# Cyan4973/FiniteStateEntropy

Hardware: AMD Instinct MI355X
Metric: MB/s encode+decode per GPU on 32KB probagen blocks; bit-exact vs CPU ref (higher is better)
Workload: dtype u8; 1 GPU; probagen Proba14, 100000 x 32KB blocks per GPU, FSE encode+decode (one-shot calls at the reference's default limits: tableLog 11, decode maxLog 12), bit-exact check; blocks_per_gpu=100000, block_bytes=32768, codec=fse, parity=fse: roundtrip-all-blocks

## Files before the change

### finitestateentropy_amd/csrc/fse_decode.hip

```cpp
#include "internal.h"
#include <atomic>

#include "bitreader.h"

#ifndef FSE_SYM_L1
#define FSE_SYM_L1 1
#endif
#ifndef FSE_DEC_RING
#define FSE_DEC_RING 64
#endif
#define FSE_IN_RING 256
#define FSE_IN_RING_LOG 8
#define FSE_IN_CHUNK 64
#define FSE_IN_LANES (FSE_IN_CHUNK / 4)
#define FSE_IN_MIRROR 16
#ifndef FSE_CHECK_EVERY
#define FSE_CHECK_EVERY 16
#endif
#ifndef FSE_PHASE_UNROLL
#define FSE_PHASE_UNROLL 16
#endif
#define FSE_FINISH_EVERY 2
#ifndef FSE_DEC_LDS_KB
#define FSE_DEC_LDS_KB 160
// ... 240 lines not shown
                nextOff -= FSE_IN_CHUNK;
                pend = 0;
                if (nextOff >= 0 && nextOff + 4 <= SgK) pend = gbl_load_u32(igK + nextOff);
            }
        }
#pragma unroll
        for (int l = 0; l < FSE_SRV_G; ++l) {
            if (!((fm >> l) & 1ull)) continue;
            const u32 cnt = srv_rl(avail, l), fp_g = srv_rl(fpos, l);
            const gbl_u8_ptr tg = (gbl_u8_ptr)(uintptr_t)srv_rl64(tabBits, l);
            if ((u32)lane < cnt) {
                u32 ri = fp_g + (u32)lane;
                ri = ri >= FSE_DEC_RING ? ri - FSE_DEC_RING : ri;
                const u32* const rw = (const u32*)(ldsb + (size_t)(g0 + l) * slotBytes + ringOff) + 4u * (ri >> 1) + (ri & 1u);
                uint2 rec; rec.x = rw[0]; rec.y = rw[2];
                const u32 x0 = __builtin_amdgcn_ubfe(rec.x, 1u, a.ldsLog), x1 = __builtin_amdgcn_ubfe(rec.x, 17u, a.ldsLog);
                const u32 x2 = __builtin_amdgcn_ubfe(rec.y, 1u, a.ldsLog), x3 = __builtin_amdgcn_ubfe(rec.y, 17u, a.ldsLog);
#if FSE_SYM_L1
                yq[l][0] = tg[x0]; yq[l][2] = tg[x1]; yq[l][1] = tg[x2]; yq[l][3] = tg[x3];
#else
                if (CALLER) {
                    yq[l][0] = __hip_atomic_load(tg + x0, __ATOMIC_RELAXED, __HIP_MEMORY_SCOPE_AGENT); yq[l][2] = __hip_atomic_load(tg + x1, __ATOMIC_RELAXED, __HIP_MEMORY_SCOPE_AGENT);
                    yq[l][1] = __hip_atomic_load(tg + x2, __ATOMIC_RELAXED, __HIP_MEMORY_SCOPE_AGENT); yq[l][3] = __hip_atomic_load(tg + x3, __ATOMIC_RELAXED, __HIP_MEMORY_SCOPE_AGENT);
                } else { yq[l][0] = tg[x0]; yq[l][2] = tg[x1]; yq[l][1] = tg[x2]; yq[l][3] = tg[x3]; }
#endif
            }
        }
        if (wantFlush) { ctl_store(&ctl->srvFlushed, it); }
#pragma unroll
        for (int l = 0; l < FSE_SRV_G; ++l) {
            if (!((fm >> l) & 1ull)) continue;
            const u32 cnt = srv_rl(avail, l), fl_g = srv_rl(flushed, l);
            gbl_u8_w_ptr const og = (gbl_u8_w_ptr)(uintptr_t)(srv_rl64(outBits, l) + 4ull * fl_g);
            if ((u32)lane < cnt) {
                const u32 w = yq[l][0] | (yq[l][1] << 8) | (yq[l][2] << 16) | (yq[l][3] << 24);
                gbl_store_u32(og + 4u * lane, w);
            }
        }
        if (wantFlush) { fpos += it - flushed; fpos = fpos >= FSE_DEC_RING ? fpos - FSE_DEC_RING : fpos; flushed = it; }
        TIMING(const unsigned long long sB = __builtin_readcyclecounter(); sBusy += sB - sA; sA = sB; ++nBusy;);
    }
    TIMING(if (lane == 0 && g0 == 0) { atomicAdd(&g_decTiming[5], sBusy); atomicAdd(&g_decTiming[6], sIdle); });
    if (CALLER) fse_scratch_slot_done(a, flagsSh, lane);
}

struct FseCellsRef { const u32* cells;
    DEV void get(u32 st, u32& ns, u32& nb, u32& sym) const { const u32 c = cells[st]; ns = c & 0xFFFFu; sym = (c >> 16) & 0xFFu; nb = c >> 24; } };
struct FseCellsCompact { const u16* A; const u8* syms;
    DEV void get(u32 st, u32& ns, u32& nb, u32& sym) const { const u32 c = A[st]; ns = c & 0xFFFu; nb = c >> 12; sym = syms[st]; } };
struct FseCellsRev { const u16* A; const u8* syms; u32 tl, cellShift;
    DEV void get(u32 st, u32& ns, u32& nb, u32& sym) const { const u32 i = __brev(st) >> (32u - tl); const u32 c = A[i]; nb = c & 31u; ns = __brev(c >> cellShift) >> (32u - tl); sym = syms[i]; } };
template <class Cells>
DEV u32 fse_tail_step(const Cells& t, u32& state, BitReader& r, bool fast)
{
    u32 ns, nb, sym;
    t.get(state, ns, nb, sym);
    const u32 low = fast ? r.read_fast(nb) : r.read(nb);
    state = ns + low;
    return sym;
}
template <class Cells>
DEV size_t fse_tail(const Cells& t, u32 s1, u32 s2, BitReader& r, u8* out, long op, long omax, bool fast)
{
    for (;;) {
        const int st = r.reload();
        if (!((st == BR_UNFINISHED) & (op < omax - 3))) break;
        u32 w = fse_tail_step(t, s1, r, fast);
        w |= fse_tail_step(t, s2, r, fast) << 8;
        w |= fse_tail_step(t, s1, r, fast) << 16;
        w |= fse_tail_step(t, s2, r, fast) << 24;
        __builtin_memcpy(out + op, &w, 4);
        op += 4;
    }
    for (;;) {
        if (op > omax - 2) return FERR(dstSize_tooSmall);
        out[op++] = (u8)fse_tail_step(t, s1, r, fast);
        if (r.reload() == BR_OVERFLOW) { out[op++] = (u8)fse_tail_step(t, s2, r, fast); return (size_t)op; }
        if (op > omax - 2) return FERR(dstSize_tooSmall);
        out[op++] = (u8)fse_tail_step(t, s2, r, fast);
        if (r.reload() == BR_OVERFLOW) { out[op++] = (u8)fse_tail_step(t, s1, r, fast); return (size_t)op; }
    }
}

template <bool FAST, bool TIMED, bool CALLER, bool VIEW = false>
__global__ __launch_bounds__(FSE_DEC_THREADS) void k_fse_decode(FseDecArgs a)
{
    extern __shared__ __attribute__((aligned(16))) u32 lds[];
    const int tid = threadIdx.x, lane = tid & 63, wave = tid >> 6;
    unsigned long long tBorn = 0, wBorn = 0;
    (void)tBorn; (void)wBorn;
    TIMING(tBorn = __builtin_readcyclecounter(); wBorn = wall_clock64(););
    const size_t first = (size_t)blockIdx.x * a.G;
    static_assert(FSE_DBINS % 4 == 0, "the bin lengths are read as 16-byte vectors");
    size_t nTot = a.nBlocks, q0 = first;
    u32 bin0 = 0, cnt0 = 0xFFFFFFFFu;
    if (a.count) {
        uint4 cv[FSE_DBINS / 4];
#pragma unroll
        for (u32 i = 0; i < FSE_DBINS / 4; ++i) cv[i] = ((const uint4*)a.count)[i];
        u64 before = 0;
        bool found = false;
#pragma unroll
        for (u32 i = 0; i < FSE_DBINS; ++i) {
            const uint4 v = cv[i >> 2];
            const u32 c = (i & 3u) == 0 ? v.x : (i & 3u) == 1 ? v.y : (i & 3u) == 2 ? v.z : v.w;
            const bool here = !found & (((u64)first < before + c) | (i == FSE_DBINS - 1));
            bin0 = here ? i : bin0; q0 = here ? (size_t)((u64)first - before) : q0; cnt0 = here ? c : cnt0;
            found |= here;
            before += c;
        }
        nTot = (size_t)before;
    }
    if (first >= nTot) return;
    auto slotBlock = [&](size_t g) -> size_t {
        if (!a.list) return first + g;
        size_t q = q0 + g; u32 i = bin0;
        if (q >= cnt0) {
            while (i < FSE_DBINS - 1) { const u32 c = a.count[i]; if (q < c) break; q -= c; ++i; }
        }
        return a.list[(size_t)i * a.nBlocks + q];
    };
    u8* const lds8 = (u8*)lds;
    const u32 tabStride = 2u << a.ldsLog;
    DecCtl* const ctlAll = (DecCtl*)(lds8 + (size_t)a.G * tabStride);
    u8* const ldsb = (u8*)ctlAll + (size_t)a.G * sizeof(DecCtl);
    const u32 slotBytes = a.slotU32 * 4u;
    const u32 ringOff = 0;
    const u32 inOff = FSE_DEC_RING * 8;

    u32* const flagsSh = (u32*)(ldsb + (size_t)a.G * slotBytes);
    if (tid < 6 || tid == 7) flagsSh[tid] = 0;
    const bool decWave = wave < FSE_DEC_WAVES;
    u8* const tlSh = (u8*)(flagsSh + 8);
    if (CALLER) {
        __syncthreads();
        bool mine = false;
        if (tid >= 64 && tid < 64 + a.G) {
            const size_t g = (size_t)tid - 64;
            u32 tl = 0xFFu;
            if (first + g < nTot) {
                const size_t bi = slotBlock(g);
                if (!(a.onlyDeclined && a.results[bi] != FSE_DECLINED)) {
                    const u32 t0 = a.dtables[bi * a.dtStrideU32] & 0xFFFFu;
                    if (t0 <= a.ldsLog && t0 >= a.tlMin) tl = t0;
                    else if (t0 > a.maxTableLog && a.tlMin == 0 && !a.onlyDeclined) a.results[bi] = FERR(tableLog_tooLarge);
                }
            }
            tlSh[g] = (u8)tl;
            mine = tl != 0xFFu;
        }
        if (mine) flagsSh[1] = 1u;
        u32 slot = 0;
        if (tid == 0) slot = fse_scratch_slot_claim(a, flagsSh);
        __syncthreads();
        if (!flagsSh[1]) {
            if (tid == 0) __hip_atomic_fetch_and(a.slotBitmap + (slot >> 5), ~(1u << (slot & 31u)), __ATOMIC_RELEASE, __HIP_MEMORY_SCOPE_AGENT);
            return;
        }
    }
    else __syncthreads();
    u8* const symSlot = CALLER ? a.symScratch + (size_t)flagsSh[6] * a.scratchSlotBytes : nullptr;
    {   u64 badBits = 0, declBits = 0; bool anyNb0 = false;
        if (!CALLER) {
            const size_t nTab = nTot - first < (size_t)a.G ? nTot - first : (size_t)a.G;
            if (tabStride >= 1024u) {
                const u32 ppt = tabStride >> 10;
                const u32 nPieces = (u32)nTab * ppt;
                for (u32 p = (u32)wave; p < nPieces; p += FSE_DEC_THREADS / 64) {
                    const u32 g = p / ppt, k = p - g * ppt;
                    const size_t bi = slotBlock(g);
                    const u8* const src = (const u8*)(a.atab + (bi << a.maxTableLog)) + 1024u * k + 16u * (u32)lane;
                    __builtin_amdgcn_global_load_lds((const __attribute__((address_space(1))) void*)src,
                                                     (__attribute__((address_space(3))) void*)(lds8 + 1024u * p), 16, 0, 0);
                }
            }
            else {
            uint4* const dstv = (uint4*)lds8;
            const u32 vptLog = a.ldsLog - 3u;
            const u32 nvec = (u32)nTab << vptLog;
            constexpr u32 MAXV = (FSE_MAXG * 512u / 16u + FSE_DEC_THREADS - 1) / FSE_DEC_THREADS;
            uint4 buf[MAXV];
#pragma unroll
            for (u32 k = 0; k < MAXV; ++k) {
                const u32 idx = tid + k * FSE_DEC_THREADS;
                if (idx < nvec) {
                    const size_t sl = first + (idx >> vptLog);
                    const size_t bi = slotBlock(sl - first);
                    buf[k] = ((const uint4*)(a.atab + (bi << a.maxTableLog)))[idx & ((1u << vptLog) - 1u)];
                }
            }
#pragma unroll
            for (u32 k = 0; k < MAXV; ++k) { const u32 idx = tid + k * FSE_DEC_THREADS; if (idx < nvec) dstv[idx] = buf[k]; }
            }
            if (!FAST) for (size_t g = 0; g < nTab; ++g) {
                const u32 st = a.meta[slotBlock(g)].state; anyNb0 |= st != 0 && !(st & 2u); }
        }
        else {
            const size_t nTab = nTot - first < (size_t)a.G ? nTot - first : (size_t)a.G;
            constexpr u32 QL = 2048u / 4u / 64u;
            if (!decWave) for (u32 g = (u32)wave - FSE_DEC_WAVES; g < (u32)nTab; g += FSE_SRV_WAVES) {
                const u32 tl = tlSh[g];
                if (tl == 0xFFu) continue;
                const u32 ts = 1u << tl;
                const u32* const t = a.dtables + slotBlock(g) * a.dtStrideU32;
                u8* const slotB = lds8 + (size_t)g * tabStride;
                u16* const A = (u16*)slotB;
                u8* const symOut = symSlot + ((size_t)g << a.ldsLog);
                bool bad = false, nbz = false;
                if (FAST && tl >= 4u) {
                    const u32 sR = 32u - tl;
                    const u32 qo[4] = { 0u, 1u << (tl - 1u), 1u << (tl - 2u), 3u << (tl - 2u) };
                    const u32 passes = ts > 2048u ? ts / 2048u : 1u;
                    u32 acc = 0, minNb = 15u;
                    uint4 cv[QL];
                    for (u32 h = 0; h < passes; ++h) {
#pragma unroll
                        for (u32 j = 0; j < QL; ++j) {
                            const u32 i0 = 2048u * h + 4u * ((u32)lane + 64u * j);
                            cv[j] = make_uint4(0, 0, 0, 0);
                            if (i0 < ts) __builtin_memcpy(&cv[j], t + 1 + i0, 16);
                        }
#pragma unroll
                        for (u32 j = 0; j < QL; ++j) {
                            const u32 i0 = 2048u * h + 4u * ((u32)lane + 64u * j);
                            if (i0 >= ts) continue;
                            const u32 r0 = __brev(i0) >> sR;
                            const u32 cw[4] = { cv[j].x, cv[j].y, cv[j].z, cv[j].w };
#pragma unroll
                            for (u32 q = 0; q < 4; ++q) {
                                const u32 c = cw[q], ns = c & 0xFFFFu, nb = c >> 24;
                                acc |= (ns >> tl) | ((tl - nb) >> 5) | (ns & ((1u << (nb & 31u)) - 1u));
                                minNb = nb < minNb ? nb : minNb;
                                slotB[r0 | qo[q]] = (u8)(c >> 16);
                            }
                        }
                    }
                    { for (u32 off = 16u * (u32)lane; off < ts; off += 1024u) { const uint4 v = *(const uint4*)(slotB + off); *(uint4*)(symOut + off) = v; } }
                    for (u32 h = 0; h < passes; ++h) {
                        if (passes > 1u) {
#pragma unroll
// ... 34 lines not shown
        if (badBits) { atomicOr(&flagsSh[2], (u32)badBits); atomicOr(&flagsSh[3], (u32)(badBits >> 32)); }
        if (declBits) { atomicOr(&flagsSh[4], (u32)declBits); atomicOr(&flagsSh[5], (u32)(declBits >> 32)); }
        if (anyNb0) atomicOr(&flagsSh[0], 1u);
    }
    const int ppw = (a.G + FSE_DEC_WAVES - 1) / FSE_DEC_WAVES;
    const int gsl = (decWave ? wave * ppw : 0) + (lane >> 1);
    const u32 half = (u32)lane & 1u, maskB = half ? ~0u : 0u;
    const bool inRange = (lane >> 1) < ppw && gsl < a.G && first + (size_t)gsl < nTot;
    const size_t b = inRange ? slotBlock((size_t)gsl) : 0;
    bool owner = decWave && inRange;
    u32 hdr = 0;
    if (owner && a.meta) { if (a.meta[b].state == 0) owner = false; else hdr = a.meta[b].hdrSize; }
    u32 tl = 0; bool fast = false;
    constexpr bool compact = !CALLER;
    const u32* const gtab = compact ? nullptr : a.dtables + (owner ? b : 0) * a.dtStrideU32;
    if (owner) {
        if (compact) { tl = a.meta[b].tableLog; fast = (a.meta[b].state & 2u) != 0; if (tl > a.ldsLog) { a.results[b] = FERR(tableLog_tooLarge); owner = false; } }
        else {
            const u32 h0 = gtab[0]; tl = h0 & 0xFFFFu; fast = (h0 >> 16) != 0;
            if (tlSh[gsl] == 0xFFu) owner = false;
        }
    }
    const u32* const cells = compact ? nullptr : gtab + 1;
    const u8* const syms = compact ? a.symtab + ((owner ? b : 0) << a.maxTableLog) : symSlot + ((size_t)(gsl < a.G ? gsl : 0) << a.ldsLog);
    const u32 ldsBase = (u32)(uintptr_t)(__attribute__((address_space(3))) u8*)lds8;
    if (ldsBase & (tabStride - 1)) __builtin_trap();
    const u32 tabOff = ldsBase + (u32)(gsl < a.G ? gsl : 0) * tabStride;
    const u16* const A = (const u16*)(lds8 + (tabOff - ldsBase));
    const u8* in = nullptr; size_t S = 0; u8* out = nullptr;
    const long omax = VIEW ? (long)a.dstCaps[owner ? b : 0] : (long)a.dstCapacity;
    long op = 0;
    BitReader r; r.base = nullptr; r.size = 0; r.at = 0; r.win = 0; r.used = 0;
    u32 s1 = 0, s2 = 0;
    if (owner) {
        in = view_ptr(a.csrc, b) + hdr;
        S = view_size(a.csrc, b) - hdr;
        out = VIEW ? a.dst + a.dstOffsets[b] : a.dst + b * a.dstStride;
        const size_t e = r.init(in, S);
        if (is_err(e)) { a.results[b] = e; owner = false; }
        else {
            s1 = r.read(tl); r.reload();
            s2 = r.read(tl); r.reload();
        }
    }

    __builtin_amdgcn_s_waitcnt(0x0f70);
    __syncthreads();
    const u64 badMask = (u64)flagsSh[2] | ((u64)flagsSh[3] << 32);
    const u64 declMask = (u64)flagsSh[4] | ((u64)flagsSh[5] << 32);
    const bool nb0 = flagsSh[0] != 0;
    if (CALLER && owner && a.declineNb0 && ((declMask >> gsl) & 1ull)) { if (half == 0) a.results[b] = FSE_DECLINED; owner = false; }

    const bool bulkOk = owner && S < (1ull << 28) && !((badMask >> gsl) & 1ull) && !(FAST && !compact && ((declMask >> gsl) & 1ull));
    const int Bstart = bulkOk ? (int)(8u * ((u32)r.at + 8u)) - (int)r.used : 0;
    const long groups0 = (omax - 3 - op + 3) / 4;
    bool can = bulkOk && (FAST ? Bstart >= 65 + 48 * (FSE_CHECK_EVERY - 1) : r.at >= 24 + 6 * FSE_CHECK_EVERY + 8) && groups0 >= FSE_CHECK_EVERY;
    bool can2 = FAST && bulkOk && Bstart >= 65 + 48 * (FSE_FINISH_EVERY - 1) && groups0 >= FSE_FINISH_EVERY;
    const bool everBulk = can || can2;
    BulkState bs; bs.q = 0; bs.bq = 0;
    {   const u32 st = half ? s2 : s1;
        bs.s = tabOff + 2u * (FAST ? __brev(st) >> (32u - (tl ? tl : 1u)) : st); }
    const u32 inA = (u32)((uintptr_t)in & 3u);
    const u32 R8 = 8u * (((u32)S + inA + 3u) & ~3u);
    u32 P = 0;
    long groups = 0;
    u32 iters = 0;
    int validLo = 0;
    if (everBulk) {
        const u32 B = 8u * ((u32)r.at + 8u + inA) - r.used;
        bs.q = 4u * (B >> 5) - 8u; bs.bq = B & 31u; P = R8 - B;
        groups = (omax - 3 - op + 3) >> 2;
        const int c0 = (int)((0 - ((uintptr_t)in - inA)) & (FSE_IN_CHUNK - 1));
        validLo = (((int)bs.q + 8 - 112 - c0) & ~(FSE_IN_CHUNK - 1)) + c0;
    }
    DecCtl* const ctl = ctlAll + (gsl < a.G ? gsl : 0);
    if (decWave && (lane >> 1) < ppw && gsl < a.G && half == 0) {
        ctl->pubIters = 0; ctl->pubPofs = everBulk ? bs.q + 8u : 0x80000000u;
        ctl->srvFlushed = 0; ctl->srvValidLo = 0x7FFFFFFF;
        ctl->initValidLo = validLo; ctl->S32 = (int)(S < (1ull << 31) ? S + inA : 0);
        const unsigned long long ib = (unsigned long long)(uintptr_t)(in - inA), ob = (unsigned long long)(uintptr_t)out, tb = (unsigned long long)(uintptr_t)syms;
        ctl->inLo = (u32)ib; ctl->inHi = (u32)(ib >> 32); ctl->outLo = (u32)ob; ctl->outHi = (u32)(ob >> 32); ctl->symLo = (u32)tb; ctl->symHi = (u32)(tb >> 32);
    }
    __syncthreads();
    if (!decWave) { fse_decode_service<TIMED, CALLER>(a, ldsb, ctlAll, slotBytes, ringOff, inOff, lane, (wave - FSE_DEC_WAVES) * FSE_SRV_G, FAST, flagsSh); return; }

    __builtin_amdgcn_s_setprio(3);
    uint2* const myRing = (uint2*)(ldsb + (size_t)(gsl < a.G ? gsl : 0) * slotBytes + ringOff) + half;
    const u32 myIn = (u32)(uintptr_t)(__attribute__((address_space(3))) u8*)(ldsb + (size_t)(gsl < a.G ? gsl : 0) * slotBytes + inOff);
    unsigned long long tRun = 0, tWait = 0, nRun = 0, nWait = 0, tA = 0, tFin = 0, nFin = 0, tInner = 0;
    (void)tRun; (void)tWait; (void)nRun; (void)nWait; (void)tA; (void)tFin; (void)nFin; (void)tInner;
    TIMING(tA = __builtin_readcyclecounter(););
    const unsigned long long tBulk0 = tA;
    (void)tBulk0;
    u32 rpos = 0;
    u64 srvNext = ctl_peek2(&ctl->srvFlushed);
    const u32 inA8 = 8u * inA;
    u32 Phead = P;
    int grp = groups > (1 << 30) ? (1 << 30) : (int)groups;
    if constexpr (FAST) {
        uint2* const dummyRing = (uint2*)(flagsSh + 32) + half;
        if ((lane >> 1) < ppw && everBulk) {
        for (;;) {
            const int lowest = (int)bs.q - 4 * ((48 * (FSE_CHECK_EVERY - 1) + 31) / 32);
            const int need = lowest > 0 ? lowest : 0;
            bool rdy;
            do {
                const u32 fl = (u32)srvNext;
                const int vlo = (int)(u32)(srvNext >> 32);
                srvNext = ctl_peek2(&ctl->srvFlushed);
                rdy = !can | ((iters + FSE_CHECK_EVERY - fl <= FSE_DEC_RING) & (need >= vlo));
                TIMING(if (!__all(rdy)) { const unsigned long long tB = __builtin_readcyclecounter(); tWait += tB - tA; ++nWait; tA = tB; });
            } while (!__all(rdy));
            if (!__any(can)) break;
            uint2* const ring = can ? myRing + rpos : dummyRing;
            u32 sN = bs.s, Pn = P, PhN = Phead;
            unsigned long long tI = 0; (void)tI;
            TIMING(tI = __builtin_readcyclecounter(););
            fse_bulk_phase_rev<FSE_CHECK_EVERY>(sN, Pn, PhN, tl + 1u, 4u, tabOff, myIn, maskB & 31u, ring);
            TIMING(tInner += __builtin_readcyclecounter() - tI;);
            bs.s = can ? sN : bs.s; P = can ? Pn : P; Phead = can ? PhN : Phead;
            const u32 adv = can ? (u32)FSE_CHECK_EVERY : 0u;
            rpos = (rpos + adv) & (FSE_DEC_RING - 1);
            iters += adv; grp -= (int)adv;
            const u32 B = R8 - P;
            bs.q = 4u * (B >> 5) - 8u;
            const u32 Bp = B - inA8;
            const bool canN = can & (Bp >= 65u + 48u * (FSE_CHECK_EVERY - 1)) & (grp >= FSE_CHECK_EVERY);
            const bool more = canN | ((Bp >= 65u + 48u * (FSE_FINISH_EVERY - 1)) & (grp >= FSE_FINISH_EVERY));
            if (can & (half == 0)) ctl_store2(&ctl->pubIters, iters, more ? bs.q + 8u : ((bs.q + 8u) | 0x80000000u));
            can = canN;
            TIMING(const unsigned long long tB = __builtin_readcyclecounter(); tRun += tB - tA; ++nRun; tA = tB;);
        }
        {   const u32 B = R8 - P; bs.bq = B & 31u;
            can2 = bulkOk & (B - inA8 >= 65u + 48u * (FSE_FINISH_EVERY - 1)) & (grp >= FSE_FINISH_EVERY); }
        can2 = can2 & bulkOk;
        for (;;) {
            const u32 fl = (u32)srvNext;
            const int vlo = (int)(u32)(srvNext >> 32);
            srvNext = ctl_peek2(&ctl->srvFlushed);
            const int lowest = (int)bs.q - 8;
            const bool rdy = !can2 | ((iters + FSE_FINISH_EVERY - fl <= FSE_DEC_RING) & ((lowest > 0 ? lowest : 0) >= vlo));
            if (!__all(rdy)) {
                TIMING(const unsigned long long tB = __builtin_readcyclecounter(); tWait += tB - tA; ++nWait; tA = tB;);
                continue;
            }
            if (!__any(can2)) break;
            uint2* const ring = can2 ? myRing + rpos : dummyRing;
            u32 sN = bs.s, Pn = P, PhN = Phead;
            fse_bulk_phase_rev<FSE_FINISH_EVERY>(sN, Pn, PhN, tl + 1u, 4u, tabOff, myIn, maskB & 31u, ring);
            bs.s = can2 ? sN : bs.s; P = can2 ? Pn : P; Phead = can2 ? PhN : Phead;
            rpos = can2 ? (rpos + FSE_FINISH_EVERY) & (FSE_DEC_RING - 1) : rpos;
            iters += can2 ? FSE_FINISH_EVERY : 0u; grp -= can2 ? FSE_FINISH_EVERY : 0;
            const u32 B = R8 - P;
            bs.q = 4u * (B >> 5) - 8u; bs.bq = B & 31u;
            const bool can2N = can2 & (B - inA8 >= 65u + 48u * (FSE_FINISH_EVERY - 1)) & (grp >= FSE_FINISH_EVERY);
            if (can2 & (half == 0)) ctl_store2(&ctl->pubIters, iters, can2N ? bs.q + 8u : ((bs.q + 8u) | 0x80000000u));
            can2 = can2N;
            TIMING(const unsigned long long tB = __builtin_readcyclecounter(); tFin += tB - tA; ++nFin; tA = tB;);
        }
        }
    } else {
    while (__any(can)) {
        const u32 fl = (u32)srvNext;
        const int vlo = (int)(u32)(srvNext >> 32);
        srvNext = ctl_peek2(&ctl->srvFlushed);
        const int lowest = (int)bs.q - (6 * FSE_CHECK_EVERY + 8);
        const bool ready = can & (iters + FSE_CHECK_EVERY - fl <= FSE_DEC_RING) & ((lowest > 0 ? lowest : 0) >= vlo);
        if (ready) {
            uint2* const ring = myRing + rpos;
            rpos = (rpos + FSE_CHECK_EVERY) & (FSE_DEC_RING - 1);
            if (nb0) fse_bulk_phase<true>(bs.s, bs.q, bs.bq, tabOff, myIn, half, maskB, ring);
            else     fse_bulk_phase<false>(bs.s, bs.q, bs.bq, tabOff, myIn, half, maskB, ring);
            iters += FSE_CHECK_EVERY; grp -= FSE_CHECK_EVERY;
            can = (bs.q >= 24u + 6u * FSE_CHECK_EVERY + 4u) & (grp >= FSE_CHECK_EVERY);
            if (half == 0) ctl_store2(&ctl->pubIters, iters, can ? bs.q + 8u : ((bs.q + 8u) | 0x80000000u));
        }
        TIMING(const unsigned long long tB = __builtin_readcyclecounter(); if (__any(ready)) { tRun += tB - tA; ++nRun; } else { tWait += tB - tA; ++nWait; } tA = tB;);
    }
    }
    TIMING(if (lane == 0) { atomicAdd(&g_decTiming[0], tRun); atomicAdd(&g_decTiming[1], tWait); atomicAdd(&g_decTiming[2], nRun); atomicAdd(&g_decTiming[3], nWait); atomicAdd(&g_decTiming[4], 1ull);
                            atomicAdd(&g_decTiming[13], tBulk0 - tBorn); atomicAdd(&g_decTiming[15], tFin); atomicAdd(&g_decTiming[10], nFin); atomicAdd(&g_decTiming[7], tInner); });
    const u32 sOther = dpp_swap(bs.s);
    const unsigned long long tBulk1 = tA;
    (void)tBulk1;
    if (owner && !half) {
    op = 4 * (long)iters;
    if (iters) {
        const u32 B = 8u * (bs.q + 8u) + bs.bq - 8u * inA;
        const u32 Bh = FAST ? R8 - Phead - 8u * inA : B;
        r.at = (size_t)((Bh + 7u) >> 3) - 8; r.used = 8u * ((u32)r.at + 8u) - B; r.win = ldg64u(in + r.at); s1 = (bs.s - tabOff) >> 1; s2 = (sOther - tabOff) >> 1;
        if (FAST) { s1 = __brev(s1) >> (32u - tl); s2 = __brev(s2) >> (32u - tl); }
    }

    size_t result;
    if (!compact) {
        if ((badMask >> gsl) & 1ull) result = fse_tail(FseCellsRef{cells}, s1, s2, r, out, op, omax, fast);
        else if (FAST)               result = fse_tail(FseCellsRev{A, syms, tl, 5u}, s1, s2, r, out, op, omax, fast);
        else                         result = fse_tail(FseCellsCompact{A, syms}, s1, s2, r, out, op, omax, fast);
    }
    else if (FAST)    result = fse_tail(FseCellsRev{A, syms, tl, 5u}, s1, s2, r, out, op, omax, fast);
    else              result = fse_tail(FseCellsCompact{A, syms}, s1, s2, r, out, op, omax, fast);
    a.results[b] = result;
    TIMING(if (lane == 0) { const unsigned long long tE = __builtin_readcyclecounter(); atomicAdd(&g_decTiming[11], tE - tBorn); atomicAdd(&g_decTiming[12], wall_clock64() - wBorn);
                            atomicAdd(&g_decTiming[14], tE - tBulk1); });
    }
    if (CALLER) fse_scratch_slot_done(a, flagsSh, lane);
}

static void fse_decode_geometry(unsigned ldsLog, size_t ldsBytes, unsigned* slotU32, int* G)
{
    *slotU32 = (FSE_DEC_RING * 8 + FSE_IN_RING + FSE_IN_MIRROR + 16) / 4;
    int g = (int)((ldsBytes - 256) / ((2u << ldsLog) + *slotU32 * 4 + sizeof(DecCtl)));
    if (g > FSE_MAXG) g = FSE_MAXG;
    *G = g;
}
#define FSE_DEC_LDS (FSE_DEC_LDS_KB * 1024)
size_t fse_decode_blocks_per_round(unsigned maxTableLog)
{
    unsigned slot; int G;
    fse_decode_geometry(maxTableLog < FSE_DEC_FAST_MAXLOG ? maxTableLog : FSE_DEC_FAST_MAXLOG, FSE_DEC_LDS, &slot, &G);
    const int cus = dev_props().ok ? dev_props().cus : 256;
    return (size_t)G * FSE_WGS_PER_CU * cus;
}

#define FSE_SYM_SLOT_BYTES (FSE_MAXG * 2048u)
#include <mutex>
namespace {
std::mutex g_symMutex;
struct SymScratch { u8* base = nullptr; u32* bitmap = nullptr; u32 nSlots = 0; };
SymScratch g_symScratch[64];
}
static hipError_t fse_sym_scratch(FseDecArgs& a, hipStream_t s)
{
    int dev = 0;
    hipError_t e = hipGetDevice(&dev);
    if (e != hipSuccess) return e;
    if (dev < 0 || dev >= 64) return hipErrorInvalidDevice;
    std::lock_guard<std::mutex> lock(g_symMutex);
    SymScratch& sc = g_symScratch[dev];
    if (!sc.base && s) {
        hipStreamCaptureStatus st = hipStreamCaptureStatusNone;
        if (hipStreamIsCapturing(s, &st) == hipSuccess && st != hipStreamCaptureStatusNone) return hipErrorStreamCaptureUnsupported;
        (void)hipGetLastError();
    }
    if (!sc.base) {
        const u32 nSlots = 2u * (u32)(dev_props().ok ? dev_props().cus : 256);
        const size_t bitmapBytes = ((nSlots + 31u) / 32u * 4u + 255u) & ~(size_t)255;
        u8* p = nullptr;
        e = hipMalloc((void**)&p, bitmapBytes + (size_t)nSlots * FSE_SYM_SLOT_BYTES);
        if (e != hipSuccess) return e;
        e = hipMemset(p, 0, bitmapBytes);
        if (e != hipSuccess) { (void)hipFree(p); return e; }
        sc.bitmap = (u32*)p; sc.base = p + bitmapBytes; sc.nSlots = nSlots;
    }
    a.symScratch = sc.base; a.slotBitmap = sc.bitmap; a.nSlots = sc.nSlots; a.scratchSlotBytes = FSE_SYM_SLOT_BYTES;
    return hipSuccess;
}

static hipError_t fse_decode_launch(FseDecArgs a, bool rev, hipStream_t s)
{
    const size_t ldsBytes = FSE_DEC_LDS;
    const bool caller = a.atab == nullptr;
    {   hipError_t e = ensure_dyn_lds((const void*)k_fse_decode<true, false, false>, FSE_DEC_LDS);
        if (e == hipSuccess) e = ensure_dyn_lds((const void*)k_fse_decode<false, false, false>, FSE_DEC_LDS);
        if (e == hipSuccess) e = ensure_dyn_lds((const void*)k_fse_decode<true, true, false>, FSE_DEC_LDS);
        if (e == hipSuccess && caller) e = ensure_dyn_lds((const void*)k_fse_decode<true, false, true>, FSE_DEC_LDS);
        if (e == hipSuccess && caller) e = ensure_dyn_lds((const void*)k_fse_decode<false, false, true>, FSE_DEC_LDS);
        if (e == hipSuccess && caller) e = fse_sym_scratch(a, s);
        if (e != hipSuccess) return e;
    }
    fse_decode_geometry(a.ldsLog, ldsBytes, &a.slotU32, &a.G);
    if (a.G < 1) return hipErrorInvalidValue;
    if (caller && ((size_t)a.G << a.ldsLog) > FSE_SYM_SLOT_BYTES) return hipErrorInvalidValue;
    const size_t groups = (a.nBlocks + a.G - 1) / a.G;
    if (a.dstOffsets) {
        if (caller || !a.dstCaps) return hipErrorInvalidValue;
        hipError_t e = ensure_dyn_lds((const void*)k_fse_decode<true, false, false, true>, FSE_DEC_LDS);
        if (e == hipSuccess) e = ensure_dyn_lds((const void*)k_fse_decode<false, false, false, true>, FSE_DEC_LDS);
        if (e != hipSuccess) return e;
        if (rev) hipLaunchKernelGGL((k_fse_decode<true, false, false, true>), dim3((unsigned)groups), dim3(FSE_DEC_THREADS), ldsBytes, s, a);
        else     hipLaunchKernelGGL((k_fse_decode<false, false, false, true>), dim3((unsigned)groups), dim3(FSE_DEC_THREADS), ldsBytes, s, a);
        return hipGetLastError();
    }
    if (caller) {
        if (rev && g_decTimingOn.load(std::memory_order_relaxed)) {
            hipError_t e = ensure_dyn_lds((const void*)k_fse_decode<true, true, true>, FSE_DEC_LDS);
            if (e != hipSuccess) return e;
            hipLaunchKernelGGL((k_fse_decode<true, true, true>), dim3((unsigned)groups), dim3(FSE_DEC_THREADS), ldsBytes, s, a);
        }
        else if (rev) hipLaunchKernelGGL((k_fse_decode<true, false, true>), dim3((unsigned)groups), dim3(FSE_DEC_THREADS), ldsBytes, s, a);
        else     hipLaunchKernelGGL((k_fse_decode<false, false, true>), dim3((unsigned)groups), dim3(FSE_DEC_THREADS), ldsBytes, s, a);
    }
    else if (rev && g_decTimingOn.load(std::memory_order_relaxed)) hipLaunchKernelGGL((k_fse_decode<true, true, false>), dim3((unsigned)groups), dim3(FSE_DEC_THREADS), ldsBytes, s, a);
    else if (rev) hipLaunchKernelGGL((k_fse_decode<true, false, false>), dim3((unsigned)groups), dim3(FSE_DEC_THREADS), ldsBytes, s, a);
    else          hipLaunchKernelGGL((k_fse_decode<false, false, false>), dim3((unsigned)groups), dim3(FSE_DEC_THREADS), ldsBytes, s, a);
    return hipGetLastError();
}

extern "C" __attribute__((visibility("default"))) int FSEHIP_prepareDevice(void)
{
    FseDecArgs a = FseDecArgs();
    return (int)fse_sym_scratch(a, nullptr);
}

extern "C" __attribute__((visibility("default"))) int FSEHIP_debug_decodeTiming(int enable, unsigned long long* out16)
{
    hipError_t e = hipDeviceSynchronize();
    if (e != hipSuccess) return (int)e;
    if (enable) {
        unsigned long long zero[16] = { 0 };
        e = hipMemcpyToSymbol(HIP_SYMBOL(g_decTiming), zero, sizeof(zero));
        g_decTimingOn.store(e == hipSuccess);
        return (int)e;
    }
    g_decTimingOn.store(false);
    if (!out16) return 0;
    e = hipMemcpyFromSymbol(out16, HIP_SYMBOL(g_decTiming), sizeof(g_decTiming));
    if (e != hipSuccess) return (int)e;
    int dev = 0, khz = 0;
    (void)hipGetDevice(&dev);
    (void)hipDeviceGetAttribute(&khz, hipDeviceAttributeClockRate, dev);
    unsigned slot; int G;
    fse_decode_geometry(FSE_DEC_FAST_MAXLOG, FSE_DEC_LDS, &slot, &G);
    out16[8] = (unsigned long long)khz; out16[9] = (unsigned long long)G | ((unsigned long long)FSE_WGS_PER_CU << 32) | ((unsigned long long)FSE_DEC_WAVES << 40) | ((unsigned long long)FSE_CHECK_EVERY << 48);
    return 0;
}

hipError_t launch_fse_decode(FseDecArgs a, hipStream_t s)
{
    if (a.nBlocks == 0) return hipSuccess;
    a.list = nullptr; a.count = nullptr;
    probe_before(PK_FSE_DECODE, s);
    a.ldsLog = a.maxTableLog < FSE_DEC_FAST_MAXLOG ? a.maxTableLog : FSE_DEC_FAST_MAXLOG;
    a.tlMin = 0; a.declineNb0 = 0; a.onlyDeclined = 0;
    hipError_t e = fse_decode_launch(a, true, s);
    if (e == hipSuccess && a.maxTableLog > FSE_DEC_FAST_MAXLOG) {
        a.ldsLog = a.maxTableLog; a.tlMin = FSE_DEC_FAST_MAXLOG + 1; a.declineNb0 = 1;
        e = fse_decode_launch(a, true, s);
        if (e == hipSuccess) { a.tlMin = 0; a.declineNb0 = 0; a.onlyDeclined = 1; e = fse_decode_launch(a, false, s); }
    }
    probe_after(PK_FSE_DECODE, s);
    return e;
}

hipError_t launch_fse_decode_classes(FseDecArgs a, const u32* lists, const u32* counts, hipStream_t s)
{
    if (a.nBlocks == 0) return hipSuccess;
    probe_before(PK_FSE_DECODE, s);
    hipError_t e = hipSuccess;
    for (int c = 0; c < FSE_DCLS_KINDS && e == hipSuccess; ++c) {
        if (c != FSE_DCLS_REV11 && a.maxTableLog <= FSE_DEC_FAST_MAXLOG) break;
        a.list = lists + (size_t)c * FSE_DBINS * a.nBlocks; a.count = counts + c * FSE_DBINS;
        a.ldsLog = c == FSE_DCLS_REV11 ? (a.maxTableLog < FSE_DEC_FAST_MAXLOG ? a.maxTableLog : FSE_DEC_FAST_MAXLOG) : a.maxTableLog;
        e = fse_decode_launch(a, c != FSE_DCLS_PLAIN, s);
    }
    probe_after(PK_FSE_DECODE, s);
    return e;
}
```

### finitestateentropy_amd/csrc/internal.h

```cpp
#pragma once
#include "dev_common.h"

#define CK(x) do { hipError_t e__ = (x); if (e__ != hipSuccess) return (int)e__; } while (0)
static inline size_t align_up(size_t v, size_t a) { return (v + a - 1) / a * a; }

static inline BlockView mkview(const void* base, size_t stride, const size_t* sizes, size_t uniform)
{
    BlockView v; v.base = (const u8*)base; v.stride = stride; v.sizes = sizes; v.uniform = uniform; v.offsets = nullptr; return v;
}
static inline BlockView subview(const BlockView& v, size_t b0)
{
    BlockView r = v;
    if (v.offsets) r.offsets = v.offsets + b0; else r.base = v.base + b0 * v.stride;
    r.sizes = v.sizes ? v.sizes + b0 : nullptr;
    return r;
}

struct HistArgs {
    unsigned* counts;
    unsigned* maxSVs;
    unsigned uniformMaxSV;
    int useUniformIn;
    int trustInput = 0;
    size_t* results;
// ... 43 lines not shown
    BlockView src;
    const u32* ctables; size_t ctStrideU32;
    const FseMeta* meta;
    unsigned maxTableLog;
    int G;
    unsigned slotU32;
    size_t nBlocks;
    unsigned onlyState;
    unsigned sizeSplit;
    u32* list; u32* count;
};
enum { FSE_EBINS = 4 };
enum { FSE_ENC_PAR = 1, FSE_ENC_LANE = 2 };
#define FSE_ENC_WAVE_MIN 2048u
__host__ __device__ inline bool fse_enc_skip(unsigned state, unsigned onlyState) { return state == 0 || (onlyState != 0 && state != onlyState); }
hipError_t launch_fse_encode(FseEncArgs a, hipStream_t s);
size_t fse_encode_blocks_per_round(unsigned maxTableLog);
hipError_t launch_fse_encode_wave(FseEncArgs a, hipStream_t s);
hipError_t launch_fse_enc_lists(const FseEncArgs& a, hipStream_t s);
inline hipError_t launch_fse_encode_auto(FseEncArgs a, hipStream_t s)
{
    a.onlyState = 0; a.sizeSplit = 0;
    const bool ragged = a.src.sizes || a.src.offsets;
    if (a.dstCapacity > 0x7FFFFFF0u || (!ragged && a.src.uniform < FSE_ENC_WAVE_MIN)) return launch_fse_encode(a, s);
    if (!a.meta) {
        a.list = nullptr; a.count = nullptr;
        if (!ragged) return launch_fse_encode_wave(a, s);
        a.sizeSplit = 1;
        const hipError_t e = launch_fse_encode_wave(a, s);
        return e != hipSuccess ? e : launch_fse_encode(a, s);
    }
    a.onlyState = FSE_ENC_PAR;
    hipError_t e = a.list ? launch_fse_enc_lists(a, s) : hipSuccess;
    if (e == hipSuccess) e = launch_fse_encode_wave(a, s);
    if (e != hipSuccess) return e;
    a.onlyState = FSE_ENC_LANE;
    return launch_fse_encode(a, s);
}

#ifndef FSE_DBINS_N
#define FSE_DBINS_N 16
#define FSE_DBIN_LOG 11
#endif
enum { FSE_DCLS_REV11 = 0, FSE_DCLS_REV12 = 1, FSE_DCLS_PLAIN = 2, FSE_DCLS_KINDS = 3, FSE_DBINS = FSE_DBINS_N, FSE_DCLS_COUNT = FSE_DCLS_KINDS * FSE_DBINS };
struct FseDPrepArgs {
    BlockView csrc;
    unsigned maxLog;
    u16* atab;
    u8* symtab;
    s16* norms;
    FseMeta* meta;
    u32* lists;
    u32* counts;
    size_t* results;
    size_t nBlocks;
    int rawRle; const size_t* origSizes; size_t uniformOrig;
};
hipError_t launch_fse_dprep(const FseDPrepArgs& a, hipStream_t s);
hipError_t launch_fse_dprep_from_norm(const FseDPrepArgs& a, const s16* norms, size_t normStride, const u32* maxSVs, u32 tl, hipStream_t s);

struct FseDecArgs {
    u8* dst; size_t dstStride; size_t dstCapacity;
    size_t* results;
    BlockView csrc;
    const u32* dtables; size_t dtStrideU32;
    const u16* atab; const u8* symtab;
    const FseMeta* meta;
    unsigned maxTableLog;
    unsigned ldsLog;
    const u32* list;
    const u32* count;
    int G;
    unsigned slotU32;
    size_t nBlocks;
    unsigned tlMin; int declineNb0; int onlyDeclined;
    u8* symScratch; u32* slotBitmap; u32 nSlots; u32 scratchSlotBytes;
    const u64* dstOffsets = nullptr; const size_t* dstCaps = nullptr;
};
#define FSE_DECLINED ((size_t)0 - (size_t)0x7001)
#define FSE_DEC_FAST_MAXLOG 11u
hipError_t launch_fse_decode(FseDecArgs a, hipStream_t s);
hipError_t launch_fse_decode_classes(FseDecArgs a, const u32* lists, const u32* counts, hipStream_t s);
size_t fse_decode_blocks_per_round(unsigned maxTableLog);

struct HufMeta {
    u32 state;
    u32 hdrSize;
    u32 tableLog;
    u32 maxSV;
};

struct HufCPrepArgs {
    const unsigned* counts; const unsigned* maxSVs; const size_t* histResults;
    BlockView src;
    u8* dst; size_t dstStride; size_t dstCapacity;
    unsigned maxSVReq, huffLogReq;
    u32* ctables; size_t ctStrideU32;
    HufMeta* meta;
    size_t* results;
    size_t nBlocks;
};
hipError_t launch_huf_cprep(const HufCPrepArgs& a, hipStream_t s, void* nodeScratch );
hipError_t launch_huf_cprep_glue(const HufCPrepArgs& a, int mode , hipStream_t s);

struct HufEncArgs {
    u8* dst; size_t dstStride; size_t dstCapacity;
    size_t* results;
    BlockView src;
    const u32* ctables; size_t ctStrideU32;
    const HufMeta* meta;
    int streams;
    int split1X;
    size_t nBlocks;
};
hipError_t launch_huf_encode(const HufEncArgs& a, hipStream_t s);

enum { HUF_DKIND_PAR_TINY = 0, HUF_DKIND_PAR_SMALL = 1, HUF_DKIND_PAR_LARGE = 2, HUF_DKIND_SERIAL = 3, HUF_DCLS_COUNT = 8 };
#ifndef HPAR_ALL_SMALL
#define HPAR_ALL_SMALL 1
#endif
#ifndef HPAR_USE_TINY
#define HPAR_USE_TINY 0
#endif
#define HPAR_DATA_TINY  2304u
#ifndef HPAR_DATA_SMALL
#define HPAR_DATA_SMALL 4608u
#endif
#define HPAR_DATA_LARGE (8192u + 384u)
#define HPAR_MIN_BITS 4096u
struct HufDPrepArgs {
    BlockView csrc;
    BlockView dstSizes;
    u8* dst; size_t dstStride;
    u32* dtables; size_t dtStrideU32;
    HufMeta* meta;
    u32* lists;
    u32* counts;
    size_t* results;
    size_t nBlocks;
    const u64* dstOffsets = nullptr;
    int tableOnly;
    unsigned dtMaxLog;
};
hipError_t launch_huf_dprep(const HufDPrepArgs& a, hipStream_t s);
hipError_t launch_huf_dprep_x2(const HufDPrepArgs& a, hipStream_t s);
hipError_t launch_hdr_results(const void* meta, size_t metaStride, size_t* results, size_t nBlocks, hipStream_t s);
hipError_t launch_fse_export_dtables(const FseDPrepArgs& a, u32* dtables, size_t dtStrideU32, hipStream_t s);

struct HufDecArgs {
    u8* dst; size_t dstStride;
    BlockView dstSizes;
    size_t* results;
    BlockView csrc;
    const u32* dtables; size_t dtStrideU32;
    const HufMeta* meta;
    unsigned maxTableLog;
    unsigned ldsLog;
    const u32* list;
    const u32* count;
    int G; unsigned slotU32;
    int streams;
    int acceptX2;
    int onlyDeclined;
    unsigned classLo;
    size_t nBlocks;
    const u64* dstOffsets = nullptr;
// ... 82 lines not shown
```

### include/fsehip.h

```cpp
#ifndef FSEHIP_H
#define FSEHIP_H

#include <stddef.h>
#include <stdint.h>

#ifdef __cplusplus
extern "C" {
#endif

#define FSEHIP_API __attribute__((visibility("default")))

typedef enum {
    FSEHIP_error_no_error = 0,
    FSEHIP_error_GENERIC = 1,
    FSEHIP_error_dstSize_tooSmall = 2,
    FSEHIP_error_srcSize_wrong = 3,
    FSEHIP_error_corruption_detected = 4,
    FSEHIP_error_tableLog_tooLarge = 5,
    FSEHIP_error_maxSymbolValue_tooLarge = 6,
    FSEHIP_error_maxSymbolValue_tooSmall = 7,
    FSEHIP_error_workSpace_tooSmall = 8,
    FSEHIP_error_maxCode = 9
} FSEHIP_ErrorCode;
#define FSEHIP_ERROR(name) ((size_t)0 - (size_t)FSEHIP_error_##name)
// ... 328 lines not shown
                                           const uint64_t* d_selFirst, size_t nSelected, void* d_scratch, size_t scratchBytes, void* stream);
FSEHIP_API int FSEHIP_tensor_patch_window_dbatch(void* d_out, uint64_t outCapacity, uint64_t* d_outOffsets, size_t* d_outResults, uint8_t* d_outCodecs,
                                                 size_t* d_tensorResults, const void* d_frames, uint64_t framesCapacity, const uint64_t* d_frameOffsets,
                                                 const size_t* d_frameResults, const uint8_t* d_codecs, const void* d_src, const void* d_base,
                                                 const uint64_t* d_srcOffsets, uint64_t capacity, const uint64_t* d_windows, size_t nTensors, unsigned elemBytes,
                                                 const uint64_t* d_segFirst, size_t nSegments, unsigned segLog, const uint64_t* d_selFirst, size_t nSelected,
                                                 const uint64_t* d_stageOffsets, uint64_t stageCapacity, size_t maxTotalBlocks, unsigned blockSizeId, int codec,
                                                 uint8_t* d_newCodecs, int policy, unsigned tolerancePermille, unsigned slotAlignLog, void* d_stage,
                                                 uint64_t* d_stagePlaneOffsets, uint64_t* d_stageSegOffsets, size_t* d_stageResults, void* d_newFrames,
                                                 uint64_t newCapacity, uint64_t* d_newOffsets, size_t* d_newResults, void* d_scratch, size_t scratchBytes,
                                                 void* d_workspace, size_t workspaceBytes, void* stream);

#define FSEHIP_DELTA_XOR 0u
#define FSEHIP_DELTA_SUB 1u
FSEHIP_API int FSEHIP_planes_split_op_dbatch(void* d_planes, uint64_t* d_planeOffsets, size_t* d_tensorResults, const void* d_src, const void* d_base,
                                             unsigned deltaOp, const uint64_t* d_srcOffsets, size_t nTensors, unsigned elemBytes, uint64_t capacity, void* stream);
FSEHIP_API int FSEHIP_planes_merge_op_dbatch(void* d_dst, const uint64_t* d_dstOffsets, size_t* d_results, const void* d_planes, const uint64_t* d_planeOffsets,
                                             const size_t* d_planeSizes, const void* d_base, unsigned deltaOp, size_t nTensors, unsigned elemBytes, uint64_t dstCapacity,
                                             void* stream);
FSEHIP_API int FSEHIP_planes_split_window_op_dbatch(void* d_stage, uint64_t* d_stagePlaneOffsets, size_t* d_stageResults, const void* d_src, const void* d_base,
                                                    unsigned deltaOp, const uint64_t* d_srcOffsets, const uint64_t* d_windows, const uint64_t* d_stageOffsets,
                                                    size_t nTensors, unsigned elemBytes, unsigned segLog, uint64_t capacity, uint64_t stageCapacity, void* stream);
FSEHIP_API int FSEHIP_tensor_compress_delta_op_dbatch(void* d_dst, uint64_t dstCapacity, uint64_t* d_frameOffsets, size_t* d_frameResults, size_t* d_tensorResults,
                                                      const void* d_src, const void* d_base, unsigned deltaOp, const uint64_t* d_srcOffsets, size_t nTensors,
                                                      unsigned elemBytes, uint64_t capacity, size_t maxTotalBlocks, unsigned blockSizeId, int codec, unsigned slotAlignLog,
                                                      void* d_planes, uint64_t* d_planeOffsets, void* d_workspace, size_t workspaceBytes, void* stream);
FSEHIP_API int FSEHIP_tensor_decompress_delta_op_dbatch(void* d_dst, const uint64_t* d_dstOffsets, uint64_t dstCapacity, const void* d_base, unsigned deltaOp,
                                                        size_t* d_results, const void* d_frames, const uint64_t* d_frameOffsets, size_t nTensors, unsigned elemBytes,
                                                        size_t maxTotalBlocks, void* d_planes, uint64_t planesCapacity, uint64_t* d_planeOffsets, size_t* d_planeResults,
                                                        void* d_workspace, size_t workspaceBytes, void* stream);
FSEHIP_API int FSEHIP_tensor_compress_mixed_op_dbatch(void* d_dst, uint64_t dstCapacity, uint64_t* d_frameOffsets, size_t* d_frameResults, size_t* d_tensorResults,
                                                      const void* d_src, const void* d_base, unsigned deltaOp, const uint64_t* d_srcOffsets, size_t nTensors,
                                                      unsigned elemBytes, uint64_t capacity, size_t maxTotalBlocks, unsigned blockSizeId, uint8_t* d_codecs, int policy,
                                                      unsigned tolerancePermille, unsigned slotAlignLog, void* d_planes, uint64_t* d_planeOffsets,
                                                      void* d_workspace, size_t workspaceBytes, void* stream);
FSEHIP_API int FSEHIP_tensor_compress_seg_op_dbatch(void* d_dst, uint64_t dstCapacity, uint64_t* d_frameOffsets, size_t* d_frameResults, size_t* d_tensorResults,
                                                    const void* d_src, const void* d_base, unsigned deltaOp, const uint64_t* d_srcOffsets, size_t nTensors,
                                                    unsigned elemBytes, uint64_t capacity, const uint64_t* d_segFirst, size_t nSegments, unsigned segLog,
                                                    size_t maxTotalBlocks, unsigned blockSizeId, int codec, uint8_t* d_codecs, int policy, unsigned tolerancePermille,
                                                    unsigned slotAlignLog, void* d_planes, uint64_t* d_planeOffsets, uint64_t* d_segOffsets, void* d_workspace,
                                                    size_t workspaceBytes, void* stream);
FSEHIP_API int FSEHIP_tensor_decompress_seg_op_dbatch(void* d_dst, const uint64_t* d_dstOffsets, uint64_t dstCapacity, const void* d_base, unsigned deltaOp,
                                                      size_t* d_results, const void* d_frames, const uint64_t* d_frameOffsets, size_t nTensors, unsigned elemBytes,
                                                      const uint64_t* d_segFirst, size_t nSegments, unsigned segLog, size_t maxTotalBlocks,
                                                      void* d_planes, uint64_t planesCapacity, uint64_t* d_segOffsets, size_t* d_segResults,
                                                      uint64_t* d_planeOffsets, size_t* d_planeSizes, void* d_workspace, size_t workspaceBytes, void* stream);
FSEHIP_API int FSEHIP_tensor_decompress_window_op_dbatch(void* d_dst, const uint64_t* d_dstOffsets, uint64_t dstCapacity, const void* d_base, unsigned deltaOp,
                                                         size_t* d_results, const void* d_frames, const uint64_t* d_frameOffsets, const uint64_t* d_srcOffsets,
                                                         const uint64_t* d_windows, size_t nTensors, unsigned elemBytes, const uint64_t* d_segFirst, size_t nSegments,
                                                         unsigned segLog, const uint64_t* d_selFirst, size_t nSelected, size_t maxTotalBlocks, void* d_planes,
                                                         uint64_t planesCapacity, uint64_t* d_selFrameOffsets, uint64_t* d_selOffsets, size_t* d_selResults,
                                                         uint64_t* d_planeOffsets, size_t* d_planeSizes, void* d_workspace, size_t workspaceBytes, void* stream);
FSEHIP_API int FSEHIP_tensor_patch_window_op_dbatch(void* d_out, uint64_t outCapacity, uint64_t* d_outOffsets, size_t* d_outResults, uint8_t* d_outCodecs,
                                                    size_t* d_tensorResults, const void* d_frames, uint64_t framesCapacity, const uint64_t* d_frameOffsets,
                                                    const size_t* d_frameResults, const uint8_t* d_codecs, const void* d_src, const void* d_base, unsigned deltaOp,
                                                    const uint64_t* d_srcOffsets, uint64_t capacity, const uint64_t* d_windows, size_t nTensors, unsigned elemBytes,
                                                    const uint64_t* d_segFirst, size_t nSegments, unsigned segLog, const uint64_t* d_selFirst, size_t nSelected,
                                                    const uint64_t* d_stageOffsets, uint64_t stageCapacity, size_t maxTotalBlocks, unsigned blockSizeId, int codec,
                                                    uint8_t* d_newCodecs, int policy, unsigned tolerancePermille, unsigned slotAlignLog, void* d_stage,
                                                    uint64_t* d_stagePlaneOffsets, uint64_t* d_stageSegOffsets, size_t* d_stageResults, void* d_newFrames,
                                                    uint64_t newCapacity, uint64_t* d_newOffsets, size_t* d_newResults, void* d_scratch, size_t scratchBytes,
                                                    void* d_workspace, size_t workspaceBytes, void* stream);

#define FSEHIP_FSEU16_MAX_SYMBOL_VALUE 286
#define FSEHIP_FSEU16_MAX_TABLELOG 13
#define FSEHIP_FSEU16_DEFAULT_TABLELOG 12
FSEHIP_API size_t FSEHIP_FSE_countU16(unsigned* count, unsigned* maxSymbolValuePtr, const unsigned short* src, size_t srcSize);
FSEHIP_API size_t FSEHIP_FSE_compressU16(void* dst, size_t dstCapacity, const unsigned short* src, size_t srcSize, unsigned maxSymbolValue, unsigned tableLog);
FSEHIP_API size_t FSEHIP_FSE_decompressU16(unsigned short* dst, size_t dstCapacity, const void* cSrc, size_t cSrcSize);
FSEHIP_API size_t FSEHIP_FSE_compressU16_batch_workspaceSize(size_t nBlocks);
FSEHIP_API size_t FSEHIP_FSE_decompressU16_batch_workspaceSize(size_t nBlocks);
FSEHIP_API int FSEHIP_FSE_countU16_batch(unsigned* d_counts, unsigned* d_maxSymbolValues, size_t* d_results, const unsigned short* d_src, size_t srcStrideBytes,
                                         const size_t* d_srcSizes, size_t uniformSrcSize, unsigned maxSymbolValue, size_t nBlocks, void* stream);
FSEHIP_API int FSEHIP_FSE_compressU16_batch(void* d_dst, size_t dstStride, size_t dstCapacity, size_t* d_results, const unsigned short* d_src, size_t srcStrideBytes,
                                            const size_t* d_srcSizes, size_t uniformSrcSize, unsigned maxSymbolValue, unsigned tableLog, size_t nBlocks,
                                            void* d_workspace, size_t workspaceBytes, void* stream);
FSEHIP_API int FSEHIP_FSE_decompressU16_batch(unsigned short* d_dst, size_t dstStrideBytes, size_t dstCapacity, size_t* d_results, const void* d_cSrc, size_t cStride,
                                              const size_t* d_cSizes, size_t uniformCSize, size_t nBlocks, void* d_workspace, size_t workspaceBytes, void* stream);

#ifdef FSEHIP_INTERNAL
FSEHIP_API int FSEHIP_probe_begin(void);
FSEHIP_API int FSEHIP_probe_collect(double* totalMs16, unsigned* launches16);
FSEHIP_API int FSEHIP_debug_decodeTiming(int enable, unsigned long long* out16);
#endif

FSEHIP_API void FSEHIP_shardRange(size_t nBlocks, int rank, int world, size_t* first, size_t* count);

#define FSEHIP_SCRATCH_BUSY (-2)
FSEHIP_API int FSEHIP_releaseScratch(void);
FSEHIP_API int FSEHIP_shutdown(void);

FSEHIP_API int FSEHIP_prepareDevice(void);

typedef struct { int deviceOrdinal; int computeUnits; int ldsBytesPerCU; int wavefrontSize; char archName[64]; } FSEHIP_DeviceInfo;
FSEHIP_API int FSEHIP_deviceInfo(FSEHIP_DeviceInfo* info);
FSEHIP_API const char* FSEHIP_versionString(void);

#ifdef FSEHIP_DROPIN_NAMES
#define HIST_count FSEHIP_HIST_count
#define FSE_compress FSEHIP_FSE_compress
#define FSE_compress2 FSEHIP_FSE_compress2
#define FSE_decompress FSEHIP_FSE_decompress
#define FSE_compress_usingCTable FSEHIP_FSE_compress_usingCTable
#define FSE_decompress_usingDTable FSEHIP_FSE_decompress_usingDTable
#define HUF_compress FSEHIP_HUF_compress
#define HUF_compress2 FSEHIP_HUF_compress2
#define HUF_decompress FSEHIP_HUF_decompress
#define HUF_compress1X_usingCTable FSEHIP_HUF_compress1X_usingCTable
#define HUF_compress4X_usingCTable FSEHIP_HUF_compress4X_usingCTable
#define HUF_decompress4X_usingDTable FSEHIP_HUF_decompress4X_usingDTable
#define HUF_decompress4X1_usingDTable FSEHIP_HUF_decompress4X1_usingDTable
#define HUF_decompress1X_usingDTable FSEHIP_HUF_decompress1X_usingDTable
#define HUF_decompress1X1_usingDTable FSEHIP_HUF_decompress1X1_usingDTable
#define HIST_count_wksp FSEHIP_HIST_count_wksp
#define HIST_countFast FSEHIP_HIST_countFast
#define HIST_countFast_wksp FSEHIP_HIST_countFast_wksp
#define HIST_count_simple FSEHIP_HIST_count_simple
#define FSE_compress_wksp FSEHIP_FSE_compress_wksp
#define FSE_decompress_wksp FSEHIP_FSE_decompress_wksp
#define HUF_compress4X_wksp FSEHIP_HUF_compress4X_wksp
#define HUF_compress1X_wksp FSEHIP_HUF_compress1X_wksp
#define HUF_compress1X FSEHIP_HUF_compress1X
#define HUF_decompress4X1_DCtx_wksp FSEHIP_HUF_decompress4X1_DCtx_wksp
#endif
#ifdef FSEHIP_DROPIN_GLUE_NAMES
#define FSE_optimalTableLog FSEHIP_FSE_optimalTableLog
#define FSE_normalizeCount FSEHIP_FSE_normalizeCount
#define FSE_NCountWriteBound FSEHIP_FSE_NCountWriteBound
#define FSE_writeNCount FSEHIP_FSE_writeNCount
#define FSE_readNCount FSEHIP_FSE_readNCount
#define FSE_buildCTable FSEHIP_FSE_buildCTable
#define FSE_buildCTable_wksp FSEHIP_FSE_buildCTable_wksp
#define FSE_buildDTable FSEHIP_FSE_buildDTable
#define HUF_buildCTable FSEHIP_HUF_buildCTable
#define HUF_buildCTable_wksp FSEHIP_HUF_buildCTable_wksp
#define HUF_writeCTable FSEHIP_HUF_writeCTable
#define HUF_readDTableX1 FSEHIP_HUF_readDTableX1
#define HUF_readDTableX1_wksp FSEHIP_HUF_readDTableX1_wksp
#define HUF_decompress4X1 FSEHIP_HUF_decompress4X1
#define HUF_decompress4X1_DCtx FSEHIP_HUF_decompress4X1_DCtx
#define HUF_decompress1X1 FSEHIP_HUF_decompress1X1
#define HUF_decompress1X1_DCtx FSEHIP_HUF_decompress1X1_DCtx
#define HUF_decompress1X1_DCtx_wksp FSEHIP_HUF_decompress1X1_DCtx_wksp
#define HUF_readDTableX2 FSEHIP_HUF_readDTableX2
#define HUF_readDTableX2_wksp FSEHIP_HUF_readDTableX2_wksp
#define HUF_decompress4X2 FSEHIP_HUF_decompress4X2
#define HUF_decompress4X2_DCtx FSEHIP_HUF_decompress4X2_DCtx
#define HUF_decompress4X2_DCtx_wksp FSEHIP_HUF_decompress4X2_DCtx_wksp
#define HUF_decompress1X2 FSEHIP_HUF_decompress1X2
#define HUF_decompress1X2_DCtx FSEHIP_HUF_decompress1X2_DCtx
#define HUF_decompress1X2_DCtx_wksp FSEHIP_HUF_decompress1X2_DCtx_wksp
#define HUF_decompress4X2_usingDTable FSEHIP_HUF_decompress4X2_usingDTable
#define HUF_decompress1X2_usingDTable FSEHIP_HUF_decompress1X2_usingDTable
#endif
#ifdef FSEHIP_DROPIN_U16_NAMES
#define FSE_countU16 FSEHIP_FSE_countU16
#define FSE_compressU16 FSEHIP_FSE_compressU16
#define FSE_decompressU16 FSEHIP_FSE_decompressU16
#endif

#ifdef __cplusplus
}
#endif
#endif
```

Measured before the change: 209,300 MiB/s of uncompressed data through encode+decode (whole job).

## Make FSE decode kernel persistent with grid-stride loop over block groups

Turns the decode kernel body into a per-group device function and wraps it in a grid-stride loop, capping the grid at the resident workgroup count (CUs times workgroups per CU) for the non-caller path. The aim is to cut workgroup launch and teardown overhead and tail effects across many small groups. It adds a __syncthreads between groups, resets wave priority at the end of each group, and adds a debug hook to override the grid cap. The risk is lost dynamic load balancing, since groups are now assigned statically round-robin instead of by the hardware dispatcher, and LDS or flag state may carry over between iterations.

Result: no change. 208,600 MiB/s of uncompressed data through encode+decode (whole job) (-0.3%).

```diff
diff --git a/finitestateentropy_amd/csrc/fse_decode.hip b/finitestateentropy_amd/csrc/fse_decode.hip
--- a/finitestateentropy_amd/csrc/fse_decode.hip
+++ b/finitestateentropy_amd/csrc/fse_decode.hip
@@ -346,15 +346,15 @@
     }
 }
 
-template <bool FAST, bool TIMED, bool CALLER, bool VIEW = false>
-__global__ __launch_bounds__(FSE_DEC_THREADS) void k_fse_decode(FseDecArgs a)
+template <bool FAST, bool TIMED, bool CALLER, bool VIEW>
+DEV bool fse_decode_group(const FseDecArgs& a, const size_t group)
 {
     extern __shared__ __attribute__((aligned(16))) u32 lds[];
     const int tid = threadIdx.x, lane = tid & 63, wave = tid >> 6;
     unsigned long long tBorn = 0, wBorn = 0;
     (void)tBorn; (void)wBorn;
     TIMING(tBorn = __builtin_readcyclecounter(); wBorn = wall_clock64(););
-    const size_t first = (size_t)blockIdx.x * a.G;
+    const size_t first = group * a.G;
     static_assert(FSE_DBINS % 4 == 0, "the bin lengths are read as 16-byte vectors");
     size_t nTot = a.nBlocks, q0 = first;
     u32 bin0 = 0, cnt0 = 0xFFFFFFFFu;
@@ -375,7 +375,7 @@
         }
         nTot = (size_t)before;
     }
-    if (first >= nTot) return;
+    if (first >= nTot) return false;
     auto slotBlock = [&](size_t g) -> size_t {
         if (!a.list) return first + g;
         size_t q = q0 + g; u32 i = bin0;
@@ -419,7 +419,7 @@
         __syncthreads();
         if (!flagsSh[1]) {
             if (tid == 0) __hip_atomic_fetch_and(a.slotBitmap + (slot >> 5), ~(1u << (slot & 31u)), __ATOMIC_RELEASE, __HIP_MEMORY_SCOPE_AGENT);
-            return;
+            return true;
         }
     }
     else __syncthreads();
@@ -620,7 +620,7 @@
         ctl->inLo = (u32)ib; ctl->inHi = (u32)(ib >> 32); ctl->outLo = (u32)ob; ctl->outHi = (u32)(ob >> 32); ctl->symLo = (u32)tb; ctl->symHi = (u32)(tb >> 32);
     }
     __syncthreads();
-    if (!decWave) { fse_decode_service<TIMED, CALLER>(a, ldsb, ctlAll, slotBytes, ringOff, inOff, lane, (wave - FSE_DEC_WAVES) * FSE_SRV_G, FAST, flagsSh); return; }
+    if (!decWave) { fse_decode_service<TIMED, CALLER>(a, ldsb, ctlAll, slotBytes, ringOff, inOff, lane, (wave - FSE_DEC_WAVES) * FSE_SRV_G, FAST, flagsSh); return true; }
 
     __builtin_amdgcn_s_setprio(3);
     uint2* const myRing = (uint2*)(ldsb + (size_t)(gsl < a.G ? gsl : 0) * slotBytes + ringOff) + half;
@@ -743,6 +743,15 @@
                             atomicAdd(&g_decTiming[14], tE - tBulk1); });
     }
     if (CALLER) fse_scratch_slot_done(a, flagsSh, lane);
+    __builtin_amdgcn_s_setprio(0);
+    return true;
+}
+
+template <bool FAST, bool TIMED, bool CALLER, bool VIEW = false>
+__global__ __launch_bounds__(FSE_DEC_THREADS) void k_fse_decode(FseDecArgs a)
+{
+    for (size_t group = blockIdx.x; fse_decode_group<FAST, TIMED, CALLER, VIEW>(a, group); group += gridDim.x)
+        __syncthreads();
 }
 
 static void fse_decode_geometry(unsigned ldsLog, size_t ldsBytes, unsigned* slotU32, int* G)
@@ -810,7 +819,13 @@
     fse_decode_geometry(a.ldsLog, ldsBytes, &a.slotU32, &a.G);
     if (a.G < 1) return hipErrorInvalidValue;
     if (caller && ((size_t)a.G << a.ldsLog) > FSE_SYM_SLOT_BYTES) return hipErrorInvalidValue;
-    const size_t groups = (a.nBlocks + a.G - 1) / a.G;
+    size_t groups = (a.nBlocks + a.G - 1) / a.G;
+    if (!caller) {
+        const unsigned cap = fse_debug_grid_cap();
+        const DevProps& dp = dev_props();
+        const size_t resident = cap ? cap : (size_t)(dp.ok ? dp.cus : 256) * FSE_WGS_PER_CU;
+        if (groups > resident) groups = resident;
+    }
     if (a.dstOffsets) {
         if (caller || !a.dstCaps) return hipErrorInvalidValue;
         hipError_t e = ensure_dyn_lds((const void*)k_fse_decode<true, false, false, true>, FSE_DEC_LDS);
@@ -864,6 +879,13 @@
     return 0;
 }
 
+static std::atomic<unsigned> g_decGridCap{0};
+unsigned fse_debug_grid_cap() { return g_decGridCap.load(std::memory_order_relaxed); }
+extern "C" __attribute__((visibility("default"))) unsigned FSEHIP_debug_decodeGrid(unsigned n)
+{
+    return g_decGridCap.exchange(n);
+}
+
 hipError_t launch_fse_decode(FseDecArgs a, hipStream_t s)
 {
     if (a.nBlocks == 0) return hipSuccess;
diff --git a/finitestateentropy_amd/csrc/internal.h b/finitestateentropy_amd/csrc/internal.h
--- a/finitestateentropy_amd/csrc/internal.h
+++ b/finitestateentropy_amd/csrc/internal.h
@@ -149,6 +149,7 @@
 hipError_t launch_fse_decode(FseDecArgs a, hipStream_t s);
 hipError_t launch_fse_decode_classes(FseDecArgs a, const u32* lists, const u32* counts, hipStream_t s);
 size_t fse_decode_blocks_per_round(unsigned maxTableLog);
+unsigned fse_debug_grid_cap();
 
 struct HufMeta {
     u32 state;
diff --git a/include/fsehip.h b/include/fsehip.h
--- a/include/fsehip.h
+++ b/include/fsehip.h
@@ -434,6 +434,7 @@
 FSEHIP_API int FSEHIP_probe_begin(void);
 FSEHIP_API int FSEHIP_probe_collect(double* totalMs16, unsigned* launches16);
 FSEHIP_API int FSEHIP_debug_decodeTiming(int enable, unsigned long long* out16);
+FSEHIP_API unsigned FSEHIP_debug_decodeGrid(unsigned n);
 #endif
 
 FSEHIP_API void FSEHIP_shardRange(size_t nBlocks, int rank, int world, size_t* first, size_t* count);
```
